# jgrodzki/radix_sort

Measured on AMD Instinct MI355X. Metric: Gkeys/sec (u64), higher is better.
Workload: dtype u64

## Files before the change

radix_sort_amd/csrc/rsx_small_kernel.hpp:

```cpp
#pragma once
#include "rsx_device.hpp"

namespace rsx {

struct SmallArgs {
    const void* src;
    void* data;
    uint32_t n;
    uint32_t passes;
    uint32_t rank_atomic;
    uint32_t map_load;
    uint32_t map_store;
    DigitSpec spec[16];
    KeyXform xf;
    const uint32_t* top_tot;
    uint32_t cap;
    uint32_t no_skip;
    uint32_t group_shift;
    uint32_t key_offset, key_bytes;
    uint32_t* hint;
};

struct PassPlan {
    uint32_t first, end;
    uint32_t mask[8];
    uint32_t low[8];
    __device__ __forceinline__ void set_masks(const uint32_t key_offset, const uint32_t key_bytes) {
#pragma unroll
        for (int w = 0; w < 8; ++w) {
            uint32_t m = 0, l = 0;
#pragma unroll
            for (uint32_t b = 0; b < 4; ++b) {
                const uint32_t byte = 4u * (uint32_t)w + b;
                if (byte >= key_offset + first && byte < key_offset + key_bytes) m |= 0xFFu << (8u * b);
                if (byte >= key_offset && byte < key_offset + first) l |= 0xFFu << (8u * b);
            }
            mask[w] = m;
            low[w] = l;
        }
    }
};

#ifndef RSX_MEND_SLACK
#define RSX_MEND_SLACK 6u
#endif
__device__ __forceinline__ uint32_t first_digit_for(const uint32_t m, const uint32_t variable_bits, const uint32_t end) {
    const uint32_t lg = m <= 1u ? 0u : 32u - (uint32_t)__builtin_clz(m - 1u);
    const uint32_t need = 2u * lg > RSX_MEND_SLACK ? 2u * lg - RSX_MEND_SLACK : 0u;
    uint32_t first = variable_bits > need ? (variable_bits - need) >> 3 : 0u;
    if (first + 1u > end) first = end != 0u ? end - 1u : 0u;
    return first;
}

template <int ES>
struct WaveCnt {
    static constexpr bool HALF = false;
    using T = typename std::conditional<HALF, uint16_t, uint32_t>::type;
    static __device__ __forceinline__ void zero(T* my, uint32_t lane) {
        uint32_t* w = reinterpret_cast<uint32_t*>(my);
#pragma unroll
        for (int i = 0; i < (HALF ? 2 : 4); ++i) w[i * WAVE + lane] = 0;
    }
    static __device__ __forceinline__ uint32_t add_rtn(T* my, uint32_t d, uint32_t v) {
        if constexpr (HALF) {
            const uint32_t sh = (d & 1u) * 16u;
            return (atomicAdd(reinterpret_cast<uint32_t*>(my) + (d >> 1), v << sh) >> sh) & 0xFFFFu;
        } else {
            return atomicAdd(&my[d], v);
        }
    }
};
template <int ES, int KPT, int WG>
__host__ __device__ constexpr uint32_t cape() {
    constexpr uint32_t slots = (uint32_t)WG * KPT;
    constexpr uint32_t room = ((163840u - 1024u - (uint32_t)(WG / WAVE) * RADIX * (uint32_t)sizeof(typename WaveCnt<ES>::T) - 64u - 3u * RADIX * 4u) / (uint32_t)ES) & ~3u;
    return slots < room ? slots : room;
}

template <int ES, int KPT, int WG>
__device__ __forceinline__ void local_load(const SmallArgs& a, const Elem<ES>* __restrict__ src, const uint32_t n, Elem<ES> (&e)[KPT]) {
    const uint32_t tid = threadIdx.x, lane = tid & 63u, wave = tid >> 6;
    const uint32_t kp = (n + WG - 1) / WG;
    const uint32_t seg = wave * (WAVE * kp) + lane;
#pragma unroll
    for (int j = 0; j < KPT; ++j) {
        e[j] = Elem<ES>{};
        if ((uint32_t)j < kp) {
            const uint32_t p = seg + (uint32_t)j * WAVE;
            if (p < n) {
                e[j] = src[p];
                if (a.map_load) key_map<ES, false>(e[j], a.xf);
            }
        }
    }
}

template <int ES, int KPT, int WG>
__device__ __forceinline__ void local_passes(const SmallArgs& a, Elem<ES> (&e)[KPT], const uint32_t n, unsigned char* smem,
                                             const uint32_t first = 0, const uint32_t end = ~0u) {
    const uint32_t stop = end == ~0u ? a.passes : end;
    constexpr int NWAVE = WG / WAVE;
    using E = Elem<ES>;
    E* s_elems = reinterpret_cast<E*>(smem);
    using C = WaveCnt<ES>;
    typename C::T* s_cnt = reinterpret_cast<typename C::T*>(smem + (size_t)cape<ES, KPT, WG>() * sizeof(E));
    uint32_t* s_misc = reinterpret_cast<uint32_t*>(s_cnt + NWAVE * RADIX);
    const uint32_t tid = threadIdx.x, lane = tid & 63u, wave = tid >> 6;
    const uint32_t kp = (n + WG - 1) / WG;
    const uint32_t seg = wave * (WAVE * kp) + lane;
    typename C::T* my = s_cnt + wave * RADIX;
    for (uint32_t pass = first; pass < stop; ++pass) {
        const DigitSpec spec = a.spec[pass];
        C::zero(my, lane);
        auto digit_of = [&](int j) -> uint32_t {
            return (seg + (uint32_t)j * WAVE >= n) ? 255u : elem_digit<ES, false>(e[j], spec);
        };
        uint32_t rk[KPT];
#pragma unroll
        for (int j = 0; j < KPT; ++j) {
            rk[j] = 0;
            if ((uint32_t)j < kp) {
                const uint32_t d = digit_of(j);
                if (a.rank_atomic) {
                    rk[j] = C::add_rtn(my, d, 1u);
                } else {
                    const uint64_t m = match_digit(d);
                    const uint32_t below = mbcnt64(m);
                    const uint32_t seen = my[d];
                    if (below == 0) (void)C::add_rtn(my, d, (uint32_t)__popcll(m));
                    rk[j] = seen + below;
                }
            }
        }
        __syncthreads();
        uint32_t tcount = 0, incl = 0;
        if (tid < RADIX) {
#pragma unroll
            for (int w = 0; w < NWAVE; ++w) tcount += s_cnt[w * RADIX + tid];
            incl = wave_incl_scan<true>(tcount);
            if (lane == 63) s_misc[wave] = incl;
        }
        __syncthreads();
        if (tid < RADIX) {
            uint32_t run = incl - tcount;
            for (uint32_t w = 0; w < wave; ++w) run += s_misc[w];
#pragma unroll
            for (int w = 0; w < NWAVE; ++w) {
                const uint32_t c = s_cnt[w * RADIX + tid];
                s_cnt[w * RADIX + tid] = (typename C::T)run;
                run += c;
            }
        }
        __syncthreads();
#pragma unroll
        for (int j = 0; j < KPT; ++j)
            if ((uint32_t)j < kp) {
                if constexpr (cape<ES, KPT, WG>() < (uint32_t)WG * KPT) {
                    if (seg + (uint32_t)j * WAVE < n) s_elems[(uint32_t)my[digit_of(j)] + rk[j]] = e[j];
                } else {
                    s_elems[(uint32_t)my[digit_of(j)] + rk[j]] = e[j];
                }
            }
        __syncthreads();
        if (pass + 1 < stop) {
#pragma unroll
            for (int j = 0; j < KPT; ++j)
                if ((uint32_t)j < kp) e[j] = s_elems[seg + (uint32_t)j * WAVE];
        }
    }
}

template <int ES, int KPT, int WG>
__device__ __forceinline__ void local_store(const SmallArgs& a, Elem<ES>* __restrict__ dst, const uint32_t n, unsigned char* smem) {
    const Elem<ES>* s_elems = reinterpret_cast<const Elem<ES>*>(smem);
    for (uint32_t i = threadIdx.x; i < n; i += WG) {
        Elem<ES> x = s_elems[i];
        if (a.map_store) key_map<ES, true>(x, a.xf);
        dst[i] = x;
    }
}

template <int ES, int KPT, int WG>
__device__ __forceinline__ void local_sort(const SmallArgs& a, const Elem<ES>* __restrict__ src, Elem<ES>* __restrict__ dst,
                                           const uint32_t n, unsigned char* smem) {
    Elem<ES> e[KPT];
    local_load<ES, KPT, WG>(a, src, n, e);
    local_passes<ES, KPT, WG>(a, e, n, smem);
    local_store<ES, KPT, WG>(a, dst, n, smem);
}

template <int ES, int KPT, int WG, typename DigitFn>
__device__ __forceinline__ void stream_pass(const SmallArgs& a, const Elem<ES>* __restrict__ src, Elem<ES>* __restrict__ dst, const uint32_t m,
                                            unsigned char* smem, DigitFn digit, const bool map_back, uint32_t& bin_start, uint32_t& bin_count) {
    constexpr int NWAVE = WG / WAVE;
    constexpr uint32_t CH = cape<ES, KPT, WG>();
    using E = Elem<ES>;
    E* s_elems = reinterpret_cast<E*>(smem);
    using C = WaveCnt<ES>;
    typename C::T* s_cnt = reinterpret_cast<typename C::T*>(smem + (size_t)cape<ES, KPT, WG>() * sizeof(E));
    uint32_t* s_misc = reinterpret_cast<uint32_t*>(s_cnt + NWAVE * RADIX);
    uint32_t* s_gbase = s_misc + NWAVE;
    uint32_t* s_dstart = s_gbase + RADIX;
    uint32_t* s_dcount = s_dstart + RADIX;
    const uint32_t tid = threadIdx.x, lane = tid & 63u, wave = tid >> 6;
    typename C::T* my = s_cnt + wave * RADIX;
    if (tid < RADIX) s_gbase[tid] = 0;
    __syncthreads();
    for (uint32_t i = tid; i < m; i += WG) atomicAdd(&s_gbase[digit(src[i])], 1u);
    __syncthreads();
    if (tid < RADIX) {
        const uint32_t c = s_gbase[tid];
        const uint32_t incl = wave_incl_scan<true>(c);
        if (lane == 63) s_misc[wave] = incl;
        s_dcount[tid] = incl - c;
        bin_count = c;
    }
    __syncthreads();
    if (tid < RADIX) {
        uint32_t b = s_dcount[tid];
        for (uint32_t w = 0; w < wave; ++w) b += s_misc[w];
        s_gbase[tid] = b;
        bin_start = b;
    }
    __syncthreads();
    for (uint32_t c0 = 0; c0 < m; c0 += CH) {
        const uint32_t n = m - c0 < CH ? m - c0 : CH;
        const uint32_t kp = (n + WG - 1) / WG;
        const uint32_t seg = wave * (WAVE * kp) + lane;
        E e[KPT];
#pragma unroll
        for (int j = 0; j < KPT; ++j) {
            e[j] = E{};
            if ((uint32_t)j < kp) {
                const uint32_t p = seg + (uint32_t)j * WAVE;
                if (p < n) e[j] = src[c0 + p];
            }
        }
        C::zero(my, lane);
        auto digit_of = [&](int j) -> uint32_t { return (seg + (uint32_t)j * WAVE >= n) ? 255u : digit(e[j]); };
        uint32_t rk[KPT];
#pragma unroll
        for (int j = 0; j < KPT; ++j) {
            rk[j] = 0;
            if ((uint32_t)j < kp) {
                const uint32_t d = digit_of(j);
                const uint64_t mm = match_digit(d);
                const uint32_t below = mbcnt64(mm);
                const uint32_t seen = my[d];
                if (below == 0) (void)C::add_rtn(my, d, (uint32_t)__popcll(mm));
                rk[j] = seen + below;
            }
        }
        __syncthreads();
        uint32_t tcount = 0, incl = 0;
        if (tid < RADIX) {
#pragma unroll
            for (int w = 0; w < NWAVE; ++w) tcount += s_cnt[w * RADIX + tid];
            incl = wave_incl_scan<true>(tcount);
            if (lane == 63) s_misc[wave] = incl;
        }
        __syncthreads();
        if (tid < RADIX) {
            uint32_t run = incl - tcount;
            for (uint32_t w = 0; w < wave; ++w) run += s_misc[w];
            s_dstart[tid] = run;
            s_dcount[tid] = tid == RADIX - 1 ? tcount - (kp * WG - n) : tcount;
#pragma unroll
            for (int w = 0; w < NWAVE; ++w) {
                const uint32_t c = s_cnt[w * RADIX + tid];
                s_cnt[w * RADIX + tid] = (typename C::T)run;
                run += c;
            }
        }
        __syncthreads();
#pragma unroll
        for (int j = 0; j < KPT; ++j)
            if ((uint32_t)j < kp) {
                if constexpr (cape<ES, KPT, WG>() < (uint32_t)WG * KPT) {
                    if (seg + (uint32_t)j * WAVE < n) s_elems[(uint32_t)my[digit_of(j)] + rk[j]] = e[j];
                } else {
                    s_elems[(uint32_t)my[digit_of(j)] + rk[j]] = e[j];
                }
            }
        __syncthreads();
        for (uint32_t i = tid; i < n; i += WG) {
            E x = s_elems[i];
            const uint32_t d = digit(x);
            const uint32_t pos = s_gbase[d] + (i - s_dstart[d]);
            if (map_back) key_map<ES, true>(x, a.xf);
            dst[pos] = x;
        }
        __syncthreads();
        if (tid < RADIX) s_gbase[tid] += s_dcount[tid];
        __syncthreads();
    }
    __builtin_amdgcn_fence(__ATOMIC_RELEASE, "agent");
    __syncthreads();
    __builtin_amdgcn_fence(__ATOMIC_ACQUIRE, "agent");
}

template <int ES, int KPT, int WG>
__device__ void big_bucket_sort(const SmallArgs& a, Elem<ES>* buf0, Elem<ES>* buf1, const uint32_t m, unsigned char* smem) {
    using E = Elem<ES>;
    E* src = buf0;
    E* dst = buf1;
    for (uint32_t pass = 0; pass < a.passes; ++pass) {
        const DigitSpec spec = a.spec[pass];
        uint32_t bs = 0, bc = 0;
        stream_pass<ES, KPT, WG>(a, src, dst, m, smem, [&](const E& x) { return elem_digit<ES, false>(x, spec); },
                                 pass + 1 == a.passes && a.map_store != 0, bs, bc);
        E* t = src;
        src = dst;
        dst = t;
    }
}

#define RSX_B16_WAVES(WG) ((WG) >= 512 ? 4 : 3)
template <int ES>
__device__ __forceinline__ bool agree(const PassPlan& pp, const Elem<ES>& x, const Elem<ES>& y) {
    uint32_t diff = 0;
#pragma unroll
    for (int w = 0; w < ES / 4; ++w) diff |= (x.w[w] ^ y.w[w]) & pp.mask[w];
    return diff == 0;
}
constexpr uint32_t MEND_LIST = 192;
template <int ES, int KPT, int WG>
__device__ __forceinline__ uint32_t* mend_count(unsigned char* smem) {
    return reinterpret_cast<uint32_t*>(smem + (size_t)cape<ES, KPT, WG>() * sizeof(Elem<ES>));
}
template <int ES, int KPT, int WG>
__device__ __forceinline__ bool local_check(const PassPlan& pp, const uint32_t n, unsigned char* smem, Elem<ES> (&x)[KPT], uint32_t& ties) {
    using E = Elem<ES>;
    const E* s_elems = reinterpret_cast<const E*>(smem);
    ties = 0;
    if (threadIdx.x == 0) *mend_count<ES, KPT, WG>(smem) = 0;
#pragma unroll
    for (int j = 0; j < KPT; ++j) {
        const uint32_t i = (uint32_t)j * WG + threadIdx.x;
        x[j] = E{};
        if (i < n) {
            x[j] = s_elems[i];
            const E p = s_elems[i != 0 ? i - 1 : 0];
            uint32_t diff = 0;
#pragma unroll
            for (int w = 0; w < ES / 4; ++w) diff |= (x[j].w[w] ^ p.w[w]) & pp.mask[w];
            ties |= (diff == 0 && i != 0) ? 1u << j : 0u;
        }
    }
    uint32_t work = 0;
    for (uint32_t t = ties; t != 0; t &= t - 1u) {
        const uint32_t i = (uint32_t)__builtin_ctz(t) * WG + threadIdx.x;
        const E u = s_elems[i], v = s_elems[i - 1];
#pragma unroll
        for (int w = 0; w < ES / 4; ++w) work |= (u.w[w] ^ v.w[w]) & pp.low[w];
    }
    return __syncthreads_or(work != 0 ? 1 : 0) != 0;
}
#ifndef RSX_MEND_INLINE
#define RSX_MEND_INLINE __forceinline__
#endif
template <int ES>
struct MendMasks {
    uint32_t hi[ES / 4], lo[ES / 4];
};
template <int ES>
__device__ RSX_MEND_INLINE uint32_t mend_listed(Elem<ES>* s_elems, uint32_t* s_list, uint32_t* s_flag, const uint32_t n, const uint32_t wg,
                                                          uint32_t ties, const MendMasks<ES> mm) {
    using E = Elem<ES>;
    constexpr uint32_t MAX_RUN = 48;
    auto same = [&](const E& u, const E& v) {
        uint32_t diff = 0;
#pragma unroll
        for (int w = 0; w < ES / 4; ++w) diff |= (u.w[w] ^ v.w[w]) & mm.hi[w];
        return diff == 0;
    };
    auto less = [&](const E& u, const E& v) {
#pragma unroll
        for (int w = ES / 4 - 1; w >= 0; --w) {
            const uint32_t a = u.w[w] & mm.lo[w], b = v.w[w] & mm.lo[w];
            if (a != b) return a < b;
        }
        return false;
    };
    if (threadIdx.x == 0) *s_flag = 0;
    for (uint32_t j = 0; ties != 0; ++j, ties >>= 1) {
        if (!(ties & 1u)) continue;
        const uint32_t i = j * wg + threadIdx.x;
        if (i >= 2 && same(s_elems[i - 1], s_elems[i - 2])) continue;
        const uint32_t k = atomicAdd(&s_list[0], 1u);
        if (k < MEND_LIST) s_list[1 + k] = i - 1;
    }
    __syncthreads();
    const uint32_t heads = s_list[0];
    if (heads > MEND_LIST) return 0u;
    if (threadIdx.x < heads) {
        const uint32_t i = s_list[1 + threadIdx.x];
        uint32_t len = 2;
        while (i + len < n && len <= MAX_RUN && same(s_elems[i + len], s_elems[i])) ++len;
        if (len > MAX_RUN) {
            *s_flag = 1;
        } else {
            for (uint32_t k = 1; k < len; ++k) {
                const E y = s_elems[i + k];
                uint32_t j = k;
                while (j > 0 && less(y, s_elems[i + j - 1])) {
                    s_elems[i + j] = s_elems[i + j - 1];
                    --j;
                }
                s_elems[i + j] = y;
            }
        }
    }
    __syncthreads();
    return *s_flag == 0 ? 1u : 0u;
}
template <int ES, int KPT, int WG>
__device__ __forceinline__ bool local_mend_listed(const uint32_t n, unsigned char* smem, const PassPlan& pp, uint32_t* s_flag, const uint32_t ties) {
    static_assert((WG / WAVE) * RADIX >= MEND_LIST + 1, "the list lives in the wave counters");
    MendMasks<ES> mm;
#pragma unroll
    for (int w = 0; w < ES / 4; ++w) {
        mm.hi[w] = pp.mask[w];
        mm.lo[w] = pp.low[w];
    }
    return mend_listed<ES>(reinterpret_cast<Elem<ES>*>(smem), mend_count<ES, KPT, WG>(smem), s_flag, n, (uint32_t)WG, ties, mm) != 0;
}
template <int ES, int KPT, int WG>
__device__ __forceinline__ void local_store_regs(const SmallArgs& a, Elem<ES>* __restrict__ dst, const uint32_t n, Elem<ES> (&x)[KPT]) {
#pragma unroll
    for (int j = 0; j < KPT; ++j) {
        const uint32_t i = (uint32_t)j * WG + threadIdx.x;
        if (i < n) {
            if (a.map_store) key_map<ES, true>(x[j], a.xf);
            dst[i] = x[j];
        }
    }
}

template <int ES, int KPT, int WG>
__device__ __forceinline__ bool local_mend_pairs(const PassPlan& pp, const uint32_t n, unsigned char* smem) {
    using E = Elem<ES>;
    E* s = reinterpret_cast<E*>(smem);
    uint32_t longer = 0;
#pragma nounroll
    for (uint32_t i = threadIdx.x + 1; i < n; i += WG) {
        const E x = s[i], p = s[i - 1];
        if (!agree<ES>(pp, x, p)) continue;
        bool run = false;
        if (i >= 2) run = agree<ES>(pp, s[i - 2], p);
        if (i + 1 < n) run = run || agree<ES>(pp, s[i + 1], x);
        int order = 0;
#pragma unroll
        for (int w = ES / 4 - 1; w >= 0; --w) {
            const uint32_t u = x.w[w] & pp.low[w], v = p.w[w] & pp.low[w];
            if (order == 0 && u != v) order = u < v ? -1 : 1;
        }
        if (run) {
            longer |= order != 0 ? 1u : 0u;
        } else if (order < 0) {
            s[i - 1] = x;
            s[i] = p;
        }
    }
    return __syncthreads_or((int)longer) != 0;
}

template <int ES, int KPT, int WG, bool PAIRS = false>
__device__ __forceinline__ bool local_finish(const SmallArgs& a, Elem<ES>* __restrict__ dst, const uint32_t n, unsigned char* smem, const PassPlan& pp,
                                             uint32_t* s_flag) {
    Elem<ES> x[KPT];
    uint32_t ties;
    if constexpr (PAIRS) {
        if (!local_mend_pairs<ES, KPT, WG>(pp, n, smem)) {
            const Elem<ES>* s_elems = reinterpret_cast<const Elem<ES>*>(smem);
#pragma unroll
            for (int j = 0; j < KPT; ++j) {
                const uint32_t i = (uint32_t)j * WG + threadIdx.x;
                x[j] = Elem<ES>{};
                if (i < n) x[j] = s_elems[i];
            }
            local_store_regs<ES, KPT, WG>(a, dst, n, x);
            return true;
        }
        (void)local_check<ES, KPT, WG>(pp, n, smem, x, ties);
    } else {
        if (!local_check<ES, KPT, WG>(pp, n, smem, x, ties)) {
            local_store_regs<ES, KPT, WG>(a, dst, n, x);
            return true;
        }
    }
    if (!local_mend_listed<ES, KPT, WG>(n, smem, pp, s_flag, ties)) return false;
    local_store<ES, KPT, WG>(a, dst, n, smem);
    return true;
}

template <int ES, int KPT, int WG, bool PAIRS = false>
__device__ __forceinline__ void local_sort_skip(const SmallArgs& a, const Elem<ES>* __restrict__ src, Elem<ES>* __restrict__ dst, const uint32_t n,
                                                unsigned char* smem, PassPlan& pp, uint32_t* s_flag) {
    using E = Elem<ES>;
    E e[KPT];
    local_load<ES, KPT, WG>(a, src, n, e);
    local_passes<ES, KPT, WG>(a, e, n, smem, pp.first, pp.end);
    if (pp.first == 0) {
        local_store<ES, KPT, WG>(a, dst, n, smem);
    } else if (!local_finish<ES, KPT, WG, PAIRS>(a, dst, n, smem, pp, s_flag)) {
        pp.first = 0;
        const uint32_t kp = (n + WG - 1) / WG, seg = (threadIdx.x >> 6) * (WAVE * kp) + (threadIdx.x & 63u);
#pragma unroll
        for (int j = 0; j < KPT; ++j)
            if ((uint32_t)j < kp) e[j] = reinterpret_cast<const E*>(smem)[seg + (uint32_t)j * WAVE];
        __syncthreads();
        local_passes<ES, KPT, WG>(a, e, n, smem, 0, pp.end);
        local_store<ES, KPT, WG>(a, dst, n, smem);
    }
}

template <int ES, int KPT>
__global__ __launch_bounds__(512) void rsx_small_sort_kernel(const SmallArgs a) {
    extern __shared__ __attribute__((aligned(16))) unsigned char smem[];
    local_sort<ES, KPT, 512>(a, static_cast<const Elem<ES>*>(a.src), static_cast<Elem<ES>*>(a.data), a.n, smem);
}

template <int ES, int KPT, int WG>
__global__ __launch_bounds__(WG) void rsx_bucket_sort_kernel(const SmallArgs a) {
    extern __shared__ __attribute__((aligned(16))) unsigned char smem[];
    uint64_t* s_red = reinterpret_cast<uint64_t*>(smem);
    const uint32_t tid = threadIdx.x, v = blockIdx.x;
    uint64_t c = 0;
    if (tid < RADIX) {
        c = a.top_tot[tid];
        if (tid == v) s_red[4] = c;
        if (v == 0) {
            uint64_t big = c;
#pragma unroll
            for (int o = 32; o > 0; o >>= 1) {
                const uint64_t y = __shfl_xor(big, o);
                big = y > big ? y : big;
            }
            if ((tid & 63u) == 0u) s_red[5 + (tid >> 6)] = big;
        }
        uint64_t below = tid < v ? c : 0ull;
#pragma unroll
        for (int o = 32; o > 0; o >>= 1) below += __shfl_xor(below, o);
        if ((tid & 63u) == 0u) s_red[tid >> 6] = below;
    }
    __syncthreads();
    const uint64_t start = s_red[0] + s_red[1] + s_red[2] + s_red[3];
    const uint64_t count = s_red[4];
    if (v == 0 && tid == 0) {
        uint64_t big = s_red[5];
        for (int w = 1; w < 4; ++w) big = s_red[5 + w] > big ? s_red[5 + w] : big;
        __hip_atomic_store(a.hint, big <= (uint64_t)a.cap / 4 ? 1u : big <= (uint64_t)a.cap ? 3u : 2u, __ATOMIC_RELAXED, __HIP_MEMORY_SCOPE_SYSTEM);
    }
    __syncthreads();
    if (count == 0) return;
    if (count > (uint64_t)cape<ES, KPT, WG>()) {
        big_bucket_sort<ES, KPT, WG>(a, const_cast<Elem<ES>*>(static_cast<const Elem<ES>*>(a.src)) + start,
                                     static_cast<Elem<ES>*>(a.data) + start, (uint32_t)count, smem);
        return;
    }
    if constexpr (ES < 8) {
        local_sort<ES, KPT, WG>(a, static_cast<const Elem<ES>*>(a.src) + start, static_cast<Elem<ES>*>(a.data) + start, (uint32_t)count, smem);
    } else {
        PassPlan pp;
        pp.end = a.passes;
        pp.first = a.no_skip ? 0u : first_digit_for((uint32_t)count, 8u * a.passes, a.passes);
        pp.set_masks(a.key_offset, a.key_bytes);
        uint32_t* s_flag = reinterpret_cast<uint32_t*>(reinterpret_cast<typename WaveCnt<ES>::T*>(smem + (size_t)cape<ES, KPT, WG>() * sizeof(Elem<ES>)) + (WG / WAVE) * RADIX) + (WG / WAVE);
        local_sort_skip<ES, KPT, WG>(a, static_cast<const Elem<ES>*>(a.src) + start, static_cast<Elem<ES>*>(a.data) + start, (uint32_t)count, smem, pp,
                                     s_flag);
    }
}

template <int ES, int KPT, int WG>
__global__ __launch_bounds__(WG, RSX_B16_WAVES(WG)) void rsx_bucket16_kernel(const SmallArgs a, const uint64_t* __restrict__ starts, void* scratch,
                                                                         const WidePlan* __restrict__ plan, Gate gate,
                                                                         const unsigned char* __restrict__ done, const uint32_t* __restrict__ left) {
    extern __shared__ __attribute__((aligned(16))) unsigned char smem[];
    if (!gate_open(gate)) return;
    using E = Elem<ES>;
    constexpr int NWAVE = WG / WAVE;
    uint32_t* s_flag = reinterpret_cast<uint32_t*>(reinterpret_cast<typename WaveCnt<ES>::T*>(smem + (size_t)cape<ES, KPT, WG>() * sizeof(E)) + NWAVE * RADIX) + NWAVE;
    const uint32_t gs = a.group_shift != 0 ? plan->group_shift : 0;
    const bool medium = (plan->verdict & VERDICT_MEDIUM) != 0;
    PassPlan pp;
    pp.end = gs == 0 ? plan->pass_end : plan->group_end;
    if (pp.end == 0) {
        if (a.map_store) {
            const uint64_t n = starts[65536];
            E* data = static_cast<E*>(a.data);
            for (uint64_t i = (uint64_t)blockIdx.x * WG + threadIdx.x; i < n; i += (uint64_t)gridDim.x * WG) {
                E x = data[i];
                key_map<ES, true>(x, a.xf);
                data[i] = x;
            }
        }
        return;
    }
    if (left != nullptr && __builtin_amdgcn_readfirstlane((int)__hip_atomic_load(left, __ATOMIC_RELAXED, __HIP_MEMORY_SCOPE_AGENT)) == 0) return;
    const uint32_t b_lo = plan->window_top - 15u;
    const uint32_t end_sub = pp.end;
    if (gs != 0) pp.end = (b_lo + gs + 7u) / 8u;
    {
        const uint64_t big = (uint64_t)plan->scan_max << gs;
        const uint32_t m = big < (uint64_t)cape<ES, KPT, WG>() ? (uint32_t)big : cape<ES, KPT, WG>();
        pp.first = a.no_skip ? 0u : first_digit_for(m, b_lo + gs, pp.end);
    }
    pp.set_masks(a.key_offset, a.key_bytes);
    for (uint32_t g = blockIdx.x; g < (65536u >> gs); g += gridDim.x) {
        const uint32_t b0 = g << gs;
        const uint64_t gstart = starts[b0];
        const uint64_t gcount = starts[b0 + (1u << gs)] - gstart;
        if (gcount == 0) continue;
        if (done != nullptr && done[g] != 0) continue;
        const bool whole = gs == 0 || gcount <= (uint64_t)cape<ES, KPT, WG>();
        const uint32_t nsub = whole ? 1u : 1u << gs;
        for (uint32_t sub = 0; sub < nsub; ++sub) {
            uint64_t start = gstart, count = gcount;
            if (!whole) {
                start = starts[b0 + sub];
                count = starts[b0 + sub + 1] - start;
            }
            if (count != 0) {
                E* bucket = static_cast<E*>(a.data) + start;
                if (count <= (uint64_t)cape<ES, KPT, WG>()) {
                    const uint32_t first = pp.first, end = pp.end;
                    if (!whole) {
                        pp.first = 0;
                        pp.end = end_sub;
                    }
                    local_sort_skip<ES, KPT, WG, true>(a, bucket, bucket, (uint32_t)count, smem, pp, s_flag);
                    if (!whole) {
                        pp.first = first;
                        pp.end = end;
                    }
                } else if (!medium) {
                    big_bucket_sort<ES, KPT, WG>(a, bucket, static_cast<E*>(scratch) + start, (uint32_t)count, smem);
                }
            }
            __syncthreads();
        }
    }
}

template <int ES, int KPT, int WG>
__global__ __launch_bounds__(WG, RSX_B16_WAVES(WG)) void rsx_bucket16_medium_kernel(const SmallArgs a, const uint64_t* __restrict__ starts, void* scratch,
                                                                                const WidePlan* __restrict__ plan, uint32_t cap256, uint32_t cap512,
                                                                                uint32_t cap1024, Gate gate) {
    extern __shared__ __attribute__((aligned(16))) unsigned char smem[];
    __shared__ uint32_t s_part[2];
    if (!gate_open(gate)) return;
    using E = Elem<ES>;
    constexpr int NWAVE = WG / WAVE;
    constexpr uint32_t CAPE = cape<ES, KPT, WG>();
    uint32_t* s_flag = reinterpret_cast<uint32_t*>(reinterpret_cast<typename WaveCnt<ES>::T*>(smem + (size_t)CAPE * sizeof(E)) + NWAVE * RADIX) + NWAVE;
    const uint32_t tid = threadIdx.x;
    const uint32_t form = plan->verdict & VERDICT_FORM_MASK;
    const uint64_t handled = form == VERDICT_WG256 ? cap256 : form == VERDICT_WG1024 ? cap1024 : cap512;
    const uint32_t end = plan->pass_end;
    if (end == 0) return;
    const uint32_t b_lo = plan->window_top - 15u;
    for (uint32_t b = blockIdx.x; b < 65536u; b += gridDim.x) {
        const uint64_t start = starts[b];
        const uint64_t count = starts[b + 1] - start;
        if (count <= handled) continue;
        E* bucket = static_cast<E*>(a.data) + start;
        E* scr = static_cast<E*>(scratch) + start;
        uint32_t k = 0;
        while (k < 8u && (count >> k) > (uint64_t)CAPE * 6u / 10u) ++k;
        if (k > b_lo) k = b_lo;
        const bool split = !(k == 0 || (count >> k) > (uint64_t)CAPE || count > 0xFFFFFFFFull);
        uint32_t kmask = 0, part_start = 0, part_count = (uint32_t)count;
        PassPlan pp;
        pp.end = end;
        pp.first = 0;
        if (split) {
            DigitSpec sp{};
            const uint32_t ebit = 8u * a.key_offset + b_lo - k;
            sp.word = ebit >> 5;
            sp.shift = ebit & 31u;
            kmask = (1u << k) - 1u;
            part_start = part_count = 0;
            const uint32_t km = kmask;
            stream_pass<ES, KPT, WG>(a, bucket, scr, (uint32_t)count, smem, [&](const E& x) { return elem_digit_any<ES>(x, sp) & km; }, false, part_start,
                                     part_count);
            const uint32_t keep = plan->keep + (k >= 4u ? 1u : 0u);
            pp.first = (end > keep && !a.no_skip) ? end - keep : 0;
            pp.set_masks(a.key_offset, a.key_bytes);
        }
        for (uint32_t j = 0; j <= kmask; ++j) {
            __syncthreads();
            if (tid == j) {
                s_part[0] = part_start;
                s_part[1] = part_count;
            }
            __syncthreads();
            const uint32_t off = s_part[0], cnt = s_part[1];
            if (cnt == 0) continue;
            if (split && cnt <= CAPE) {
                local_sort_skip<ES, KPT, WG>(a, scr + off, bucket + off, cnt, smem, pp, s_flag);
            } else {
                if (split) {
                    for (uint32_t i = tid; i < cnt; i += WG) bucket[off + i] = scr[off + i];
                    __builtin_amdgcn_fence(__ATOMIC_RELEASE, "agent");
                    __syncthreads();
                    __builtin_amdgcn_fence(__ATOMIC_ACQUIRE, "agent");
                }
                big_bucket_sort<ES, KPT, WG>(a, bucket + off, scr + off, cnt, smem);
            }
        }
        __syncthreads();
    }
}

constexpr uint32_t DIRECT_LIMIT = 24;
template <int WG>
__host__ __device__ constexpr uint32_t direct_bits() {
    return WG >= 1024 ? 12u : WG >= 512 ? 11u : 10u;
}
template <int ES>
__device__ __forceinline__ bool key_less(const Elem<ES>& x, const Elem<ES>& y) {
    static_assert(ES == 8 || ES == 16, "key-only elements of 8 and 16 bytes");
    if constexpr (ES == 8) {
        return (((uint64_t)x.w[1] << 32) | x.w[0]) < (((uint64_t)y.w[1] << 32) | y.w[0]);
    } else {
        const uint64_t xh = ((uint64_t)x.w[3] << 32) | x.w[2], yh = ((uint64_t)y.w[3] << 32) | y.w[2];
        const uint64_t xl = ((uint64_t)x.w[1] << 32) | x.w[0], yl = ((uint64_t)y.w[1] << 32) | y.w[0];
        return xh < yh || (xh == yh && xl < yl);
    }
}
__device__ __forceinline__ uint32_t wave_max(uint32_t x) {
    auto step = [](uint32_t v, auto ctrl, auto rows) {
        const uint32_t y = (uint32_t)__builtin_amdgcn_update_dpp(0, (int)v, decltype(ctrl)::value, decltype(rows)::value, 0xf, false);
        return y > v ? y : v;
    };
    x = step(x, std::integral_constant<int, 0x111>{}, std::integral_constant<int, 0xf>{});
    x = step(x, std::integral_constant<int, 0x112>{}, std::integral_constant<int, 0xf>{});
    x = step(x, std::integral_constant<int, 0x114>{}, std::integral_constant<int, 0xf>{});
    x = step(x, std::integral_constant<int, 0x118>{}, std::integral_constant<int, 0xf>{});
    x = step(x, std::integral_constant<int, 0x142>{}, std::integral_constant<int, 0xa>{});
    x = step(x, std::integral_constant<int, 0x143>{}, std::integral_constant<int, 0xc>{});
    return (uint32_t)__builtin_amdgcn_readlane((int)x, 63);
}
template <int ES>
__device__ __forceinline__ void direct_read(const unsigned char* smem, const uint32_t q, Elem<ES> (&y)[16 / ES]) {
    const uint4 v = reinterpret_cast<const uint4*>(smem)[q];
    if constexpr (ES == 8) {
        y[0].w[0] = v.x;
        y[0].w[1] = v.y;
        y[1].w[0] = v.z;
        y[1].w[1] = v.w;
    } else {
        y[0].w[0] = v.x;
        y[0].w[1] = v.y;
        y[0].w[2] = v.z;
        y[0].w[3] = v.w;
    }
}
template <int ES, bool EDGE>
__device__ __forceinline__ void direct_rank(const unsigned char* smem, const uint32_t q, const uint32_t M, const uint32_t n, const Elem<ES> (&x)[16 / ES],
                                            uint32_t (&r)[16 / ES]) {
    constexpr int G = 16 / ES;
    const uint32_t words = (n + G - 1) / G;
#pragma unroll 2
    for (uint32_t m = 1; m <= M; ++m) {
        Elem<ES> lo[G], hi[G];
        uint32_t ql = q - m, qh = q + m;
        bool vl = true, vh = true;
        if constexpr (EDGE) {
            vl = q >= m;
            vh = qh < words;
            ql = vl ? ql : q;
            qh = vh ? qh : q;
        }
        direct_read<ES>(smem, ql, lo);
        direct_read<ES>(smem, qh, hi);
#pragma unroll
        for (int h = 0; h < G; ++h) {
            bool okl = true, okh = true;
            if constexpr (EDGE) {
                okl = vl;
                okh = vh && qh * G + (uint32_t)h < n;
            }
#pragma unroll
            for (int g = 0; g < G; ++g) {
                r[g] -= (okl && key_less<ES>(x[g], lo[h])) ? 1u : 0u;
                r[g] += (okh && key_less<ES>(hi[h], x[g])) ? 1u : 0u;
            }
        }
    }
}

template <int ES, int KPT, int WG>
__global__ __launch_bounds__(WG, RSX_B16_WAVES(WG)) void rsx_bucket16_direct_kernel(const SmallArgs a, const uint64_t* __restrict__ starts,
                                                                                const WidePlan* __restrict__ plan, unsigned char* __restrict__ done,
                                                                                uint32_t* __restrict__ left, Gate gate) {
    extern __shared__ __attribute__((aligned(16))) unsigned char smem[];
    if (!gate_open(gate)) return;
    using E = Elem<ES>;
    constexpr int NWAVE = WG / WAVE;
    constexpr int G = 16 / ES;
    constexpr uint32_t CAPE = cape<ES, KPT, WG>();
    constexpr uint32_t B = direct_bits<WG>(), NB = 1u << B;
    static_assert(NB == (uint32_t)NWAVE * RADIX && NB == 4u * WG && sizeof(typename WaveCnt<ES>::T) == 4, "the counters take the wave counters' place, four to a thread");
    static_assert((CAPE * ES) % 16 == 0, "the counters are read and written as uint4");
    E* s = reinterpret_cast<E*>(smem);
    uint32_t* s_cnt = reinterpret_cast<uint32_t*>(smem + (size_t)CAPE * sizeof(E));
    uint32_t* s_tot = s_cnt + NB + 4;
    const uint32_t tid = threadIdx.x, lane = tid & 63u, wave = tid >> 6;
    const uint32_t b_lo = plan->window_top - 15u;
    const uint32_t bd = b_lo < B ? b_lo : B;
    const uint32_t dshift = b_lo - bd, dmask = (1u << bd) - 1u;
    const uint32_t dword = dshift >> 5, dsh = dshift & 31u;
    auto digit_of = [&](const E& x) -> uint32_t {
        const uint32_t lo = elem_word<ES>(x, dword);
        const uint32_t hi = elem_word<ES>(x, dword + 1u < (uint32_t)(ES / 4) ? dword + 1u : dword);
        return (uint32_t)(((((uint64_t)hi << 32) | lo) >> dsh)) & dmask;
    };
    auto leave_from = [&](const uint32_t g) -> uint32_t {
        uint32_t mine = 0;
        for (uint32_t b = g + tid * gridDim.x; b < 65536u; b += (uint32_t)WG * gridDim.x) {
            done[b] = 0;
            mine += starts[b + 1] != starts[b] ? 1u : 0u;
        }
        if (tid == 0) s_tot[0] = 0;
        __syncthreads();
        if (mine != 0) atomicAdd(&s_tot[0], mine);
        __syncthreads();
        return s_tot[0];
    };
    uint32_t left_here = 0;
    if (plan->pass_end == 0) {
        if (blockIdx.x < 65536u) left_here = leave_from(blockIdx.x);
        if (tid == 0 && left_here != 0) atomicAdd(left, left_here);
        return;
    }
    for (uint32_t g = blockIdx.x; g < 65536u; g += gridDim.x) {
        const uint64_t start = starts[g];
        const uint64_t count = starts[g + 1] - start;
        if (count == 0 || count > (uint64_t)CAPE) {
            if (tid == 0) done[g] = 0;
            left_here += count != 0 ? 1u : 0u;
            continue;
        }
        const uint32_t n = (uint32_t)count;
        E* bucket = static_cast<E*>(a.data) + start;
        reinterpret_cast<uint4*>(s_cnt)[tid] = uint4{0u, 0u, 0u, 0u};
        E e[KPT];
#pragma unroll
        for (int j = 0; j < KPT; ++j) {
            const uint32_t i = (uint32_t)j * WG + tid;
            e[j] = E{};
            if (i < n) e[j] = bucket[i];
        }
        __syncthreads();
        uint32_t rk[KPT];
#pragma unroll
        for (int j = 0; j < KPT; ++j) {
            rk[j] = 0;
            if ((uint32_t)j * WG + tid < n) rk[j] = atomicAdd(&s_cnt[digit_of(e[j])], 1u);
        }
        __syncthreads();
        const uint4 c = reinterpret_cast<const uint4*>(s_cnt)[tid];
        const uint32_t sum = c.x + c.y + c.z + c.w;
        const uint32_t m01 = c.x > c.y ? c.x : c.y, m23 = c.z > c.w ? c.z : c.w;
        const uint32_t incl = wave_incl_scan<true>(sum);
        if (lane == 63) s_tot[wave] = incl;
        if (__syncthreads_or((m01 > m23 ? m01 : m23) > DIRECT_LIMIT ? 1 : 0)) {
            left_here += leave_from(g);
            break;
        }
        uint32_t run = incl - sum;
        for (uint32_t w = 0; w < wave; ++w) run += s_tot[w];
        reinterpret_cast<uint4*>(s_cnt)[tid] = uint4{run, run + c.x, run + c.x + c.y, run + c.x + c.y + c.z};
        if (tid == 0) s_cnt[NB] = n;
        __syncthreads();
#pragma unroll
        for (int j = 0; j < KPT; ++j)
            if ((uint32_t)j * WG + tid < n) s[s_cnt[digit_of(e[j])] + rk[j]] = e[j];
        __syncthreads();
        const uint32_t words = (n + G - 1) / G;
        auto rank_word = [&](const uint32_t q0, const bool live, const uint32_t q, E (&x)[G], uint32_t (&r)[G]) {
            direct_read<ES>(smem, q, x);
            uint32_t need = 0;
#pragma unroll
            for (int h = 0; h < G; ++h) {
                const uint32_t p = q * G + (uint32_t)h;
                r[h] = p;
                if (live && p < n) {
                    const uint32_t d = digit_of(x[h]);
                    const uint32_t below = p - s_cnt[d], above = s_cnt[d + 1u] - 1u - p;
                    need = need > below ? need : below;
                    need = need > above ? need : above;
                }
            }
            const uint32_t T = wave_max(need);
            const uint32_t M = (T + G - 1) / G;
            if constexpr (G == 2) {
                const bool both = q * 2u + 1u < n;
                const uint32_t inv = (both && key_less<ES>(x[1], x[0])) ? 1u : 0u;
                r[0] += inv;
                r[1] -= inv;
            }
            if (q0 >= M && q0 + 63u + M < n / G) direct_rank<ES, false>(smem, q, M, n, x, r);
            else direct_rank<ES, true>(smem, q, M, n, x, r);
        };
#pragma nounroll
        for (uint32_t q0 = (uint32_t)__builtin_amdgcn_readfirstlane((int)(tid & ~63u)); q0 < words; q0 += WG) {
            const bool live = q0 + lane < words;
            const uint32_t q = live ? q0 + lane : words - 1u;
            E x[G];
            uint32_t r[G];
            rank_word(q0, live, q, x, r);
#pragma unroll
            for (int h = 0; h < G; ++h)
                if (live && q * G + (uint32_t)h < n) {
                    E y = x[h];
                    if (a.map_store) key_map<ES, true>(y, a.xf);
                    if (r[h] < n) bucket[r[h]] = y;
                }
        }
        if (tid == 0) done[g] = 1;
        __syncthreads();
    }
    if (tid == 0 && left_here != 0) atomicAdd(left, left_here);
}

}
```

Measured before the change: 77.97.

## Pack two 16-bit digit counters per word to add one direct-sort digit bit

The direct bucket kernel now stores two 16-bit counters in each 32-bit shared-memory word. This allows one extra digit bit in the same counter space. Ranking uses shifted atomic adds on the half-word, and the scan writes start offsets for both halves together. The finer digits shrink the per-digit windows that the later direct ranking has to search, and they make the fall-back to the slower path less frequent. The cost is extra unpacking arithmetic, and counters are limited to 16 bits, which a static assert guards.

```diff
diff --git a/radix_sort_amd/csrc/rsx_small_kernel.hpp b/radix_sort_amd/csrc/rsx_small_kernel.hpp
--- a/radix_sort_amd/csrc/rsx_small_kernel.hpp
+++ b/radix_sort_amd/csrc/rsx_small_kernel.hpp
@@ -713,11 +713,15 @@
     }
 }
 
+#ifndef RSX_DIRECT_PACKED
+#define RSX_DIRECT_PACKED 1
+#endif
 constexpr uint32_t DIRECT_LIMIT = 24;
 template <int WG>
 __host__ __device__ constexpr uint32_t direct_bits() {
     return WG >= 1024 ? 12u : WG >= 512 ? 11u : 10u;
 }
+constexpr uint32_t DIRECT_EXTRA_BITS = RSX_DIRECT_PACKED ? 1u : 0u;
 template <int ES>
 __device__ __forceinline__ bool key_less(const Elem<ES>& x, const Elem<ES>& y) {
     static_assert(ES == 8 || ES == 16, "key-only elements of 8 and 16 bytes");
@@ -808,8 +812,11 @@
     uint32_t* s_cnt = reinterpret_cast<uint32_t*>(smem + (size_t)CAPE * sizeof(E));
     uint32_t* s_tot = s_cnt + NB + 4;
     const uint32_t tid = threadIdx.x, lane = tid & 63u, wave = tid >> 6;
+    constexpr bool PACKED = DIRECT_EXTRA_BITS != 0;
+    constexpr uint32_t BC = B + DIRECT_EXTRA_BITS;
+    static_assert(CAPE < (1u << 16), "a count and a start fit a half");
     const uint32_t b_lo = plan->window_top - 15u;
-    const uint32_t bd = b_lo < B ? b_lo : B;
+    const uint32_t bd = b_lo < BC ? b_lo : BC;
     const uint32_t dshift = b_lo - bd, dmask = (1u << bd) - 1u;
     const uint32_t dword = dshift >> 5, dsh = dshift & 31u;
     auto digit_of = [&](const E& x) -> uint32_t {
@@ -817,6 +824,10 @@
         const uint32_t hi = elem_word<ES>(x, dword + 1u < (uint32_t)(ES / 4) ? dword + 1u : dword);
         return (uint32_t)(((((uint64_t)hi << 32) | lo) >> dsh)) & dmask;
     };
+    auto start_of = [&](const uint32_t d) -> uint32_t {
+        if constexpr (PACKED) return reinterpret_cast<const uint16_t*>(s_cnt)[d];
+        else return s_cnt[d];
+    };
     auto leave_from = [&](const uint32_t g) -> uint32_t {
         uint32_t mine = 0;
         for (uint32_t b = g + tid * gridDim.x; b < 65536u; b += (uint32_t)WG * gridDim.x) {
@@ -858,26 +869,52 @@
 #pragma unroll
         for (int j = 0; j < KPT; ++j) {
             rk[j] = 0;
-            if ((uint32_t)j * WG + tid < n) rk[j] = atomicAdd(&s_cnt[digit_of(e[j])], 1u);
+            if ((uint32_t)j * WG + tid < n) {
+                const uint32_t d = digit_of(e[j]);
+                if constexpr (PACKED) {
+                    const uint32_t sh = (d & 1u) << 4;
+                    rk[j] = (atomicAdd(&s_cnt[d >> 1], 1u << sh) >> sh) & 0xFFFFu;
+                } else {
+                    rk[j] = atomicAdd(&s_cnt[d], 1u);
+                }
+            }
         }
         __syncthreads();
         const uint4 c = reinterpret_cast<const uint4*>(s_cnt)[tid];
-        const uint32_t sum = c.x + c.y + c.z + c.w;
-        const uint32_t m01 = c.x > c.y ? c.x : c.y, m23 = c.z > c.w ? c.z : c.w;
+        uint32_t p0 = c.x, p1 = c.y, p2 = c.z, p3 = c.w;
+        uint32_t big;
+        if constexpr (PACKED) {
+            auto low = [](uint32_t v) { return v & 0xFFFFu; };
+            auto larger = [](uint32_t u, uint32_t v) { return u > v ? u : v; };
+            p0 = low(c.x) + (c.x >> 16), p1 = low(c.y) + (c.y >> 16), p2 = low(c.z) + (c.z >> 16), p3 = low(c.w) + (c.w >> 16);
+            const uint32_t pairs = larger(larger(p0, p1), larger(p2, p3));
+            const uint32_t halves = larger(larger(larger(low(c.x), c.x >> 16), larger(low(c.y), c.y >> 16)),
+                                           larger(larger(low(c.z), c.z >> 16), larger(low(c.w), c.w >> 16)));
+            big = b_lo > B ? pairs : halves;
+        } else {
+            const uint32_t m01 = c.x > c.y ? c.x : c.y, m23 = c.z > c.w ? c.z : c.w;
+            big = m01 > m23 ? m01 : m23;
+        }
+        const uint32_t sum = p0 + p1 + p2 + p3;
         const uint32_t incl = wave_incl_scan<true>(sum);
         if (lane == 63) s_tot[wave] = incl;
-        if (__syncthreads_or((m01 > m23 ? m01 : m23) > DIRECT_LIMIT ? 1 : 0)) {
+        if (__syncthreads_or(big > DIRECT_LIMIT ? 1 : 0)) {
             left_here += leave_from(g);
             break;
         }
         uint32_t run = incl - sum;
         for (uint32_t w = 0; w < wave; ++w) run += s_tot[w];
-        reinterpret_cast<uint4*>(s_cnt)[tid] = uint4{run, run + c.x, run + c.x + c.y, run + c.x + c.y + c.z};
+        if constexpr (PACKED) {
+            const uint32_t r1 = run + p0, r2 = r1 + p1, r3 = r2 + p2;
+            reinterpret_cast<uint4*>(s_cnt)[tid] = uint4{(c.x << 16) + run * 0x10001u, (c.y << 16) + r1 * 0x10001u, (c.z << 16) + r2 * 0x10001u, (c.w << 16) + r3 * 0x10001u};
+        } else {
+            reinterpret_cast<uint4*>(s_cnt)[tid] = uint4{run, run + c.x, run + c.x + c.y, run + c.x + c.y + c.z};
+        }
         if (tid == 0) s_cnt[NB] = n;
         __syncthreads();
 #pragma unroll
         for (int j = 0; j < KPT; ++j)
-            if ((uint32_t)j * WG + tid < n) s[s_cnt[digit_of(e[j])] + rk[j]] = e[j];
+            if ((uint32_t)j * WG + tid < n) s[start_of(digit_of(e[j])) + rk[j]] = e[j];
         __syncthreads();
         const uint32_t words = (n + G - 1) / G;
         auto rank_word = [&](const uint32_t q0, const bool live, const uint32_t q, E (&x)[G], uint32_t (&r)[G]) {
@@ -889,7 +926,7 @@
                 r[h] = p;
                 if (live && p < n) {
                     const uint32_t d = digit_of(x[h]);
-                    const uint32_t below = p - s_cnt[d], above = s_cnt[d + 1u] - 1u - p;
+                    const uint32_t below = p - start_of(d), above = start_of(d + 1u) - 1u - p;
                     need = need > below ? need : below;
                     need = need > above ? need : above;
                 }
```

New measurement: 79.03 (median of 6 runs). 1.01x the previous value.
